# uncbiag/DeepAtlas

Hardware: AMD Instinct MI355X
Metric: training volumes/sec at 160x192x160 fp32; Dice vs CPU ref (higher is better)
Workload: dtype f32; 1 GPU; seg-only UNet_light + softmax-Dice + Adam training step, batch 2/GPU, 160x192x160 fp32 (BASELINE configs[1]); global_batch=2, n_classes=32, parallelism=dp1, matrix_precision=fp32_split, hip_graph=False, matrix_arithmetic_bits=22

## Files before the change

deepatlas_amd/csrc/conv3d_mfma.hip:

```cpp
#include "common.h"
#include "conv3d_internal.h"
#include "split_f16.h"

#include "conv3d_stage.h"
#ifndef DA_BF16_SMAP
#ifndef DA_BF16_SMAP2
#define DA_BF16_SMAP2 0
#endif
#define DA_BF16_SMAP 1
#endif
#ifndef DA_SP_LB
#define DA_SP_LB 1
#endif
#ifndef DA_RPB4
#define DA_RPB4 0
#endif
#ifndef DA_PIN
#define DA_PIN 1
#endif

namespace {


template <int CK, int NREP, bool MASKED = false, int STATS = 0, bool BF = false, bool PRO = false, bool SP = false, int S2F = 0, bool PAIR = false, bool HB = false>
__global__ void __launch_bounds__(256, 2) conv3_mfma_fwd_kernel(FwdP p) {
    static_assert(!HB || (BF && !SP), "bf16 activation storage: bf16 matrix mode only");
    static_assert(STATS != 2 || (SP && NREP == 1 && !PRO), "BatchNorm-backward sums: the split mode's one-N-tile data gradient");
    static_assert((S2F != 0) == MASKED, "the tap-masked (stride-2) variants and only they address X / dX through the space-to-depth view");
    static_assert(!PAIR || (SP && NREP == 1 && !PRO), "paired staging: split mode, one N-tile, no input prologue");
    static_assert(!SP || (BF && !MASKED && CK == 8), "split mode: dense bf16 K = 32 kernels on 8-channel chunks");
    constexpr int NP = SP ? 2 : 1;
    constexpr bool RAW = HB && BF && !SP && !PRO && !MASKED && S2F == 0;
    extern __shared__ __attribute__((aligned(16))) float lds[];
    constexpr bool K32 = BF && !MASKED;
    using AElem = std::conditional_t<BF, short, float>;
    using Frag = std::conditional_t<SP, f16x8, std::conditional_t<K32, bf16x8, std::conditional_t<BF, s16x4, f32x4>>>;
    constexpr int EB = BF ? 2 : 4;
    constexpr int TZ = 4, HZ = TZ + 2;
    constexpr int NSTEPS = K32 ? (CK == 16 ? 14 : 7) : (27 * CK + 15) / 16;
    constexpr int NIT = StageGeom<CK, HZ>::NIT;
    constexpr int PRE = MASKED ? (NREP == 1 ? NIT : 4) : ((NREP <= 2) ? NIT : (NREP == 3 ? (NIT < 4 ? NIT : 4) : 0));
    static_assert(!PRO || (PRE == NIT && !MASKED), "the prologue variant keeps the whole next tile in registers");
    const int lane = threadIdx.x & 63;
    const int wave = __builtin_amdgcn_readfirstlane((int)(threadIdx.x >> 6));
    const int i = lane & 15, g = lane >> 4;
    const int nt0 = blockIdx.y * NREP;
    const unsigned long long clk0 = __builtin_readcyclecounter(), rt0 = __builtin_amdgcn_s_memrealtime();
    const int nchunks = (p.C1 + p.C2) / CK;
    const TileWalk tw = tile_walk(p.ntiles);
    const int nitems = tw.cnt * nchunks;
    if (nitems <= 0) {
        if (STATS) for (int c = threadIdx.x; c < NREP * 16; c += 256) { const int co = blockIdx.y * NREP * 16 + c; if (co < p.Cout) { p.stats_partial[((size_t)blockIdx.x * 2) * p.Cout + co] = 0.0; p.stats_partial[((size_t)blockIdx.x * 2 + 1) * p.Cout + co] = 0.0; } }
        return;
    }
// ... 32 lines not shown
                    if constexpr (NIT > B2) { float4 tmp[NIT - B2]; stage_load_s2d<CK, HZ, B2, NIT, HB>(tmp, p.in1, p.s2in, cbase, n, z0, y0, x0, p.D, p.H, p.W); stage_write<CK, HZ, B2, NIT, BF, SP>(lds, tmp); }
                }
            } else {
            { float4 tmp[B1 - PRE]; stage_load<CK, HZ, PRE, B1, HB, RAW>(tmp, src, Cs, choff, n, z0, y0, x0, p.D, p.H, p.W); stage_write<CK, HZ, PRE, B1, BF, SP, 0, RAW>(lds, tmp); }
            if constexpr (B2 > B1) { float4 tmp[B2 - B1]; stage_load<CK, HZ, B1, B2, HB, RAW>(tmp, src, Cs, choff, n, z0, y0, x0, p.D, p.H, p.W); stage_write<CK, HZ, B1, B2, BF, SP, 0, RAW>(lds, tmp); }
            if constexpr (NIT > B2) { float4 tmp[NIT - B2]; stage_load<CK, HZ, B2, NIT, HB, RAW>(tmp, src, Cs, choff, n, z0, y0, x0, p.D, p.H, p.W); stage_write<CK, HZ, B2, NIT, BF, SP, 0, RAW>(lds, tmp); }
            }
        }
    };

    f32x4 acc[TY][NREP];
#pragma unroll
    for (int r = 0; r < TY; ++r)
#pragma unroll
        for (int nn = 0; nn < NREP; ++nn) acc[r][nn] = (f32x4){0.f, 0.f, 0.f, 0.f};

    float st1[STATS ? NREP : 1][4], st2[STATS ? NREP : 1][4];
#pragma unroll
    for (int nn = 0; nn < (STATS ? NREP : 1); ++nn)
#pragma unroll
        for (int j = 0; j < 4; ++j) { st1[nn][j] = 0.f; st2[nn][j] = 0.f; }
    double dsum1 = 0.0, dsum2 = 0.0;
    double* sred = reinterpret_cast<double*>(reinterpret_cast<char*>(lds) + (size_t)StageGeom<CK, HZ>::TOTAL * 4 * EB * NP);
    int tiles_done = 0;
    auto stats_flush = [&]() {
        if constexpr (STATS) {
#pragma unroll
            for (int nn = 0; nn < NREP; ++nn)
#pragma unroll
                for (int j = 0; j < 4; ++j) {
                    double a = (double)st1[nn][j], b = (double)st2[nn][j];
                    a += __shfl_xor(a, 1); b += __shfl_xor(b, 1);
                    a += __shfl_xor(a, 2); b += __shfl_xor(b, 2);
                    a += __shfl_xor(a, 4); b += __shfl_xor(b, 4);
                    a += __shfl_xor(a, 8); b += __shfl_xor(b, 8);
                    if ((lane & 15) == 0) {
                        const int c = nn * 16 + 4 * (lane >> 4) + j;
                        sred[(wave * 2 + 0) * (NREP * 16) + c] = a;
                        sred[(wave * 2 + 1) * (NREP * 16) + c] = b;
                    }
                    st1[nn][j] = 0.f; st2[nn][j] = 0.f;
                }
            __syncthreads();
            if ((int)threadIdx.x < NREP * 16) {
                const int c = threadIdx.x;
#pragma unroll
                for (int w = 0; w < 4; ++w) { dsum1 += sred[(w * 2 + 0) * (NREP * 16) + c]; dsum2 += sred[(w * 2 + 1) * (NREP * 16) + c]; }
            }
            __syncthreads();
        }
    };
    float4 pre[PRE > 0 ? PRE : 1];
    float4 pre2[PAIR ? PRE : 1];
    unsigned vm = 0;
    float4 psc = make_float4(1.f, 1.f, 1.f, 1.f), psf = make_float4(0.f, 0.f, 0.f, 0.f); float pslope = -1.f;
    auto load_pro = [&](int item) {
        if constexpr (PRO) {
            int n, z0, y0, x0, ch;
            item_coords(item, n, z0, y0, x0, ch);
            const int cbase = ch * CK;
            const bool first = cbase < p.C1;
            const int cofs = (first ? cbase : cbase - p.C1) + ((int)threadIdx.x % StageGeom<CK, HZ>::Q) * 4;
            psc = *reinterpret_cast<const float4*>((first ? p.ps1 : p.ps2) + cofs);
            psf = *reinterpret_cast<const float4*>((first ? p.pt1 : p.pt2) + cofs);
            pslope = first ? p.pslope1 : p.pslope2;
// ... 76 lines not shown
        else if constexpr (BF) return __builtin_amdgcn_mfma_f32_16x16x16bf16_1k(b, a, c, 0, 0, 0);
        else return c;
    };
    constexpr int LB = SP ? (NREP == 1 ? DA_SP_LB : 1) : (NREP == 1) ? 4 : ((NREP == 2 && !STATS) ? 2 : 1);
    constexpr int RB = LB + 1;
    constexpr int TAIL = SP ? 2 : 5;
    constexpr int PRO_DELAY = SP ? 1 : 3;
    constexpr bool PRO_IN = PRO && NREP == 1;
    static_assert(!PRO || NSTEPS - TAIL + PRO_DELAY <= NSTEPS, "prologue arithmetic must fall inside the K loop");
    Frag bq[RB][NREP][NP], nb[LB][NREP][NP];
    if constexpr (!MASKED) {
#pragma unroll
        for (int t = 0; t < LB; ++t)
#pragma unroll
            for (int nn = 0; nn < NREP; ++nn)
#pragma unroll
                for (int pl = 0; pl < NP; ++pl) nb[t][nn][pl] = wb(0, t, nn, pl);
    }
    const int a4 = g;
    float bvv[NREP][4];
#pragma unroll
    for (int nn = 0; nn < NREP; ++nn)
#pragma unroll
        for (int j = 0; j < 4; ++j) { const int co = (nt0 + nn) * 16 + 4 * a4 + j; bvv[nn][j] = (p.bias && co < p.Cout) ? p.bias[co] : 0.f; }

    auto item_body = [&](int item, auto PHC) {
        constexpr int PH = decltype(PHC)::value;
        int n, z0, y0, x0, ch;
        item_coords(0, n, z0, y0, x0, ch);
        const bool has_next = PH == 1 ? true : (item + 1 < nitems);
        const bool last = (ch == nchunks - 1);
        if constexpr (SP) {
            if (Ecur != Eacc) {
                if (ch != 0) {
                    const float f = da_acc_factor(Ecur - Eacc);
#pragma unroll
                    for (int r = 0; r < TY; ++r)
#pragma unroll
                        for (int nn = 0; nn < NREP; ++nn) acc[r][nn] = acc[r][nn] * f;
                }
                Eacc = Ecur;
            }
        }

        if constexpr (MASKED) {
            const Frag* wch = reinterpret_cast<const Frag*>(p.wp) + ((size_t)ch * NSTEPS * p.NT + nt0) * 64 + lane;
            if (has_next && !(p.ablate & 1)) issue_stage(1, pre);
// ... 160 lines not shown
#pragma unroll
                for (int nn = 0; nn < NREP; ++nn)
#pragma unroll
                    for (int r = 0; r < HALF; ++r) acc[HALF + r][nn] = mma_bf(acc[HALF + r][nn], A1[r], bq[s % RB][nn][0]);
            } else {
#pragma unroll
            for (int m = 0; m < 4; ++m) {
#pragma unroll
                for (int nn = 0; nn < NREP; ++nn)
#pragma unroll
                    for (int r = 0; r < HALF; ++r)
                        acc[HALF + r][nn] = __builtin_amdgcn_mfma_f32_16x16x4f32(bq[s % RB][nn][0][m], A1[r][m], acc[HALF + r][nn], 0, 0, 0);
                if (DA_PIN) __builtin_amdgcn_sched_barrier(0);
            }
            }
        }
        }

        {
            const int z = z0 + wave;
            const int x = x0 + i;
            const bool do_ep = last && !(p.ablate & 2);
            const float inv1 = SP ? da_pow2(-(Ecur / 2)) : 1.f, inv2 = SP ? da_pow2(-(Ecur - Ecur / 2)) : 1.f;
            float4 yq[STATS == 2 ? TY : 1], bsc = make_float4(0.f, 0.f, 0.f, 0.f), bsf = bsc, bmu = bsc;
            if constexpr (STATS == 2) {
                const int cq = nt0 * 16 + 4 * a4;
                const bool cokq = do_ep && (cq + 3 < p.Cout) && z < p.D && x < p.W;
                const __amdgpu_buffer_rsrc_t ry = da_rsrc_n<false>(p.bst_y, n, (long long)p.D * p.H * p.W * p.Cs1);
#pragma unroll
                for (int r = 0; r < TY; ++r) {
                    const unsigned off = ((unsigned)((z * p.H + (y0 + r)) * p.W + x) * (unsigned)p.Cs1 + (unsigned)cq) * 4u;
                    yq[r] = da_buf_load4(ry, (cokq && y0 + r < p.H) ? off : 0xFFFFFFFFu);
                }
                const __amdgpu_buffer_rsrc_t rp = da_rsrc(p.bst_par, (unsigned)(4 * p.Cs1 * 4));
                const unsigned po = (do_ep && cq + 3 < p.Cout) ? (unsigned)(cq * 4) : 0xFFFFFFFFu;
                bmu = da_buf_load4(rp, po);
                bsc = da_buf_load4(rp, po == 0xFFFFFFFFu ? po : po + (unsigned)(2 * p.Cs1 * 4));
                bsf = da_buf_load4(rp, po == 0xFFFFFFFFu ? po : po + (unsigned)(3 * p.Cs1 * 4));
            }
            if (do_ep) {
#pragma unroll
                for (int nn = 0; nn < NREP; ++nn) {
#pragma unroll
                    for (int r = 0; r < TY; ++r) {
                        float t0 = acc[r][nn][0], t1 = acc[r][nn][1], t2 = acc[r][nn][2], t3 = acc[r][nn][3];
                        if constexpr (SP) { t0 = t0 * inv1 * inv2; t1 = t1 * inv1 * inv2; t2 = t2 * inv1 * inv2; t3 = t3 * inv1 * inv2; }
                        const float v0 = t0 + bvv[nn][0], v1 = t1 + bvv[nn][1], v2 = t2 + bvv[nn][2], v3 = t3 + bvv[nn][3];
                        if constexpr (STATS == 2) {
                            const float m = (z < p.D && y0 + r < p.H && x < p.W) ? 1.f : 0.f;
                            const float4 yv = yq[r];
                            const float d0 = m * v0 * da_act_grad(yv.x * bsc.x + bsf.x, p.bst_slope), d1 = m * v1 * da_act_grad(yv.y * bsc.y + bsf.y, p.bst_slope);
                            const float d2 = m * v2 * da_act_grad(yv.z * bsc.z + bsf.z, p.bst_slope), d3 = m * v3 * da_act_grad(yv.w * bsc.w + bsf.w, p.bst_slope);
                            st1[nn][0] += d0; st1[nn][1] += d1; st1[nn][2] += d2; st1[nn][3] += d3;
                            st2[nn][0] += d0 * (yv.x - bmu.x); st2[nn][1] += d1 * (yv.y - bmu.y); st2[nn][2] += d2 * (yv.z - bmu.z); st2[nn][3] += d3 * (yv.w - bmu.w);
                        } else if (STATS) {
                            const float m = (z < p.D && y0 + r < p.H && x < p.W) ? 1.f : 0.f;
                            st1[nn][0] += m * v0; st1[nn][1] += m * v1; st1[nn][2] += m * v2; st1[nn][3] += m * v3;
                            st2[nn][0] += m * v0 * v0; st2[nn][1] += m * v1 * v1; st2[nn][2] += m * v2 * v2; st2[nn][3] += m * v3 * v3;
                        }
                        acc[r][nn] = (f32x4){da_act(v0, p.slope), da_act(v1, p.slope), da_act(v2, p.slope), da_act(v3, p.slope)};
                        if constexpr (STATS) __builtin_amdgcn_sched_barrier(0);
                    }
                }
            }
#pragma unroll
            for (int nn = 0; nn < NREP; ++nn) {
                const int cb = (nt0 + nn) * 16;
                const bool first = cb < p.Cs1;
                float* dbase = first ? p.out1 : p.out2;
                const int Cd = first ? p.Cs1 : p.Cs2;
                const int cd = cb - (first ? 0 : p.Cs1) + 4 * a4;
                const bool cok = do_ep && (cb + 4 * a4 + 3 < p.Cout) && z < p.D && x < p.W;
                constexpr bool scattered = (S2F == 2);
                if constexpr (S2F == 2) {
                    {
                        const int rr = cb / p.s2out.cin, c0 = cb - rr * p.s2out.cin + 4 * a4;
                        const int zs = 2 * z + ((rr >> 2) & 1), xs = 2 * x + (rr & 1), ry = (rr >> 1) & 1;
                        const long long sample0 = (long long)p.s2out.D0 * p.s2out.H0 * p.s2out.W0 * p.s2out.cin;
                        const __amdgpu_buffer_rsrc_t r0 = da_rsrc_n<HB>(p.out1, n, sample0);
                        const bool ok0 = cok && zs < p.s2out.D0 && xs < p.s2out.W0;
#pragma unroll
                        for (int r = 0; r < TY; ++r) {
                            const int ys = 2 * (y0 + r) + ry;
                            const unsigned off = ((unsigned)((zs * p.s2out.H0 + ys) * p.s2out.W0 + xs) * (unsigned)(p.s2out.cin) + (unsigned)(c0)) * (unsigned)(HbEl<HB>::ES);
// ... 1368 lines not shown
    size_t pk = 0;
    if (Cin % 8 == 0) { const size_t a = packed_bytes(Cin, Cout, Cin % 16 == 0 ? 16 : 8); if (a > pk) pk = a; const size_t b = packed_bytes(Cin, Cout, 8); if (b > pk) pk = b; }
    if (Cout % 8 == 0) { const size_t a = packed_bytes(Cout, Cin, Cout % 16 == 0 ? 16 : 8); if (a > pk) pk = a; }
    size_t part = 0;
    if (Cin % 8 == 0) { part = wgrad_plan(N, D, H, W, Cin, 0, Cout).partial_bytes; const size_t pr = wgrad_plan(N, D, H, W, Cin, 0, Cout, true, true, true).partial_bytes; if (pr > part) part = pr; }
    if (Cin <= 4 && Cout <= 32) part = da_align((size_t)kScBlocksFwd * 27 * Cin * Cout * sizeof(float));
    if (Cout <= 4 && Cin <= 32) { const size_t sw = da_align((size_t)(kScBlocksFwd + 1) * 27 * Cin * Cout * sizeof(float)); if (sw > part) part = sw; }
    return pk + tile_table_bytes(N, D, H, W) + part + wg_tile_table_bytes(N, D, H, W);
}

bool da_conv3_mfma_fwd_supported(int C1, int C2, int Cout, int stride, int Cs1, int Cs2) {
    if (stride != 1) return false;
    if (pick_ck(C1, C2) == 0) return false;
    if (Cout < 8) return false;
    if (Cout % 4 != 0) return false;
    if (Cs1 < 0) { Cs1 = Cout; Cs2 = 0; }
    if (Cs2 > 0 && (Cs1 % 16 != 0 || Cs2 % 4 != 0)) return false;
    if ((unsigned long long)Cs1 % 4 != 0) return false;
    return true;
}

template <int CK, int NREP, bool MASKED = false, int STATS = 0, bool BF = false, bool PRO = false, bool SP = false, int S2F = 0, bool PAIR = false, bool HB = false>
static int launch_fwd_mfma(const FwdP& p, int gy, hipStream_t st) {
    const size_t shm = (size_t)6 * HY * HX * CK * (BF ? 2 : 4) * (SP ? 2 : 1) + (STATS ? (size_t)4 * 2 * NREP * 16 * sizeof(double) : 0) + (SP ? 16 : 0);
    auto kern = conv3_mfma_fwd_kernel<CK, NREP, MASKED, STATS, BF, PRO, SP, S2F, PAIR, HB>;
    static bool attr_set = false;
    if (!attr_set) {
        hipError_t e = hipFuncSetAttribute(reinterpret_cast<const void*>(kern), hipFuncAttributeMaxDynamicSharedMemorySize, (int)shm);
        if (e != hipSuccess) return (int)e;
        attr_set = true;
    }
    { static int occ = -1; if (occ < 0) { occ = getenv("DA_OCC") ? 1 : 0; if (occ) { int nb = 0; (void)hipOccupancyMaxActiveBlocksPerMultiprocessor(&nb, kern, 256, shm); fprintf(stderr, "[occ] <%d,%d,M%d,S%d,BF%d,PRO%d,SP%d> lds %zu B -> %d workgroups per CU\n", CK, NREP, (int)MASKED, (int)STATS, (int)BF, (int)PRO, (int)SP, shm, nb); } } }
    static unsigned long long* dclk = nullptr; static int want = -1;
    if (want < 0) { want = getenv("DA_CLK") ? 1 : 0; if (want) (void)hipMalloc(&dclk, 64 + 1024 * 16); }
    FwdP q = p; q.clk = want ? dclk : nullptr;
    if (want) { const unsigned long long init[6] = {0, 0, ~0ull, 0, ~0ull, 0}; (void)hipMemcpyAsync(dclk, init, 48, hipMemcpyHostToDevice, st); (void)hipStreamSynchronize(st); }
    hipLaunchKernelGGL(kern, dim3(p.nblocks, gy), dim3(256), shm, st, q);
    if (want) {
        unsigned long long h[6]; (void)hipStreamSynchronize(st); (void)hipMemcpy(h, dclk, 48, hipMemcpyDeviceToHost);
        fprintf(stderr, "[clk] cycles %llu realtime %llu -> %.0f MHz; grid %d x %d: starts span %.1f us, ends span %.1f us, first start -> last end %.1f us\n", h[0], h[1],
                (double)h[0] / (double)h[1] * 100.0, p.nblocks, gy, (h[3] - h[2]) * 0.01, (h[5] - h[4]) * 0.01, (h[5] - h[2]) * 0.01);
        if (getenv("DA_CLK_DUMP")) {
            static unsigned long long rec[2048];
            const int nb = p.nblocks < 1024 ? p.nblocks : 1024;
            (void)hipMemcpy(rec, dclk + 8, (size_t)nb * 16, hipMemcpyDeviceToHost);
            for (int b = 0; b < nb; ++b) fprintf(stderr, "[blk] %d xcc %llu hwid %08llx life_us %.1f\n", b, (rec[2 * b] >> 32) & 15, rec[2 * b] & 0xffffffffull, rec[2 * b + 1] * 0.01);
        }
// ... 11 lines not shown
        float* h = (float*)malloc(2 * kProMaxC * sizeof(float));
        for (int i = 0; i < kProMaxC; ++i) { h[i] = 1.f; h[kProMaxC + i] = 0.f; }
        e = hipMemcpy(buf, h, 2 * kProMaxC * sizeof(float), hipMemcpyHostToDevice);
        free(h);
        if (e != hipSuccess) return (int)e;
    }
    *ones = buf; *zeros = buf + kProMaxC;
    return 0;
}

static int pro_slopes(const DaPro* pro, int C2, float* s1, float* s2) {
    const float a = pro->s1 ? pro->slope1 : -1.f, b = (C2 > 0 && pro->s2) ? pro->slope2 : -1.f;
    if (a >= 1.f || b >= 1.f) return 1;
    *s1 = a < 0.f ? 1.f : a; *s2 = b < 0.f ? 1.f : b;
    return 0;
}

static int conv3_mfma_fwd_impl(const float* in1, int C1, const float* in2, int C2, const float* w_tio, int w_is_flipped_tr,
                               const float* bias, float* out1, int Cs1, float* out2, int Cs2,
                               int N, int D, int H, int W, int Cout, int stride, float slope,
                               void* ws, size_t ws_bytes, hipStream_t st, int s2d_cin, double* stats_partial, int* stats_nparts, const DaPro* pro, const DaS2dFuse* s2f,
                               int cout0, int CoutW, bool hb);

struct BstState { const float* y; const float* par; float slope; };
static thread_local BstState g_bst = {nullptr, nullptr, -1.f};

struct PrepackState { int mode; const float* w; char* buf[2]; size_t bytes[2]; int next, used; };
static thread_local PrepackState g_pp = {0, nullptr, {nullptr, nullptr}, {0, 0}, 0, 0};
static thread_local PackJobs* g_pp_collect = nullptr;
static thread_local int g_pp_ncollect = 0;

int da_conv3_mfma_fwd(const float* in1, int C1, const float* in2, int C2, const float* w_tio, int w_is_flipped_tr,
                      const float* bias, float* out1, int Cs1, float* out2, int Cs2,
                      int N, int D, int H, int W, int Cout, int stride, float slope,
                      void* ws, size_t ws_bytes, hipStream_t st, int s2d_cin, double* stats_partial, int* stats_nparts, const DaPro* pro, const DaS2dFuse* s2f, int act_bf16) {
    if (act_bf16 && da_matrix_mode() != 1) return DA_ERR_UNSUPPORTED;
    struct PpReset { ~PpReset() { if (g_pp.mode == 1) g_pp.mode = 0; } } pp_reset;
    if (g_pp.mode && g_pp.w != w_tio) g_pp.mode = 0;
    if (da_matrix_mode() == 2 && w_is_flipped_tr && s2d_cin == 0 && !stats_partial && !pro && Cs2 > 0 && Cs1 == 32 && Cs2 == 16 && Cout == 48 &&
        pick_ck(C1, C2) != 0) {
        int rc = conv3_mfma_fwd_impl(in1, C1, in2, C2, w_tio, 1, bias, out1, 32, nullptr, 0, N, D, H, W, 32, stride, slope, ws, ws_bytes, st, 0, nullptr, nullptr,
                                     nullptr, nullptr, 0, Cout, false);
        if (rc) return rc;
        return conv3_mfma_fwd_impl(in1, C1, in2, C2, w_tio, 1, bias ? bias + 32 : nullptr, out2, 16, nullptr, 0, N, D, H, W, 16, stride, slope, ws, ws_bytes, st, 0,
                                   nullptr, nullptr, nullptr, nullptr, 32, Cout, false);
    }
    return conv3_mfma_fwd_impl(in1, C1, in2, C2, w_tio, w_is_flipped_tr, bias, out1, Cs1, out2, Cs2, N, D, H, W, Cout, stride, slope, ws, ws_bytes, st, s2d_cin,
                               stats_partial, stats_nparts, pro, s2f, 0, Cout, act_bf16 != 0);
// ... 2 lines not shown
static int conv3_mfma_fwd_impl(const float* in1, int C1, const float* in2, int C2, const float* w_tio, int w_is_flipped_tr,
                               const float* bias, float* out1, int Cs1, float* out2, int Cs2,
                               int N, int D, int H, int W, int Cout, int stride, float slope,
                               void* ws, size_t ws_bytes, hipStream_t st, int s2d_cin, double* stats_partial, int* stats_nparts, const DaPro* pro, const DaS2dFuse* s2f,
                               int cout0, int CoutW, bool hb) {
    (void)stride;
    const int Cin = C1 + C2;
    int CK = pick_ck(C1, C2);
    if (!CK) return DA_ERR_UNSUPPORTED;
    if (pro && (s2d_cin > 0 || w_is_flipped_tr || Cin > kProMaxC)) return DA_ERR_UNSUPPORTED;
    if (s2d_cin > 0 && !s2f) return DA_ERR_UNSUPPORTED;
    const bool split = da_matrix_mode() == 2 && s2d_cin == 0;
    const bool bf = da_matrix_mode() == 1;
    if (split) CK = 8;
    {
        const unsigned long long vox4 = (unsigned long long)D * H * W * 4ull;
        const int cmax = (C1 > C2 ? C1 : C2) > (Cs1 > Cs2 ? Cs1 : Cs2) ? (C1 > C2 ? C1 : C2) : (Cs1 > Cs2 ? Cs1 : Cs2);
        if (vox4 * (unsigned long long)cmax >= 0xFFFFFFF0ull) return DA_ERR_UNSUPPORTED;
    }
    const int NT = (Cout + 15) / 16;
    int NREP = pick_nrep(NT);
    if ((bf || split || pro) && NREP > 2) NREP = 2;
    const bool want_bst = g_bst.y != nullptr && split && stats_partial != nullptr;
    if (want_bst) NREP = 1;
    {
        const long long tiles = (long long)N * ((D + 3) / 4) * ((H + TY - 1) / TY) * ((W + TX - 1) / TX);
        if (s2d_cin == 0 && NREP > 1 && !want_bst) {
            auto cost = [&](int nrep) {
                const int g = (NT + nrep - 1) / nrep;
                long long nb = 512 / g; if (nb < 1) nb = 1; if (nb > tiles) nb = tiles;
                return (double)((tiles + nb - 1) / nb) * nrep * (nrep == 1 ? 1.08 : 1.0);
            };
            if (cost(1) < cost(NREP)) NREP = 1;
        }
    }
    const int gy = (NT + NREP - 1) / NREP, NTpad = gy * NREP;
    const int pkmode = split ? 3 : bf ? (s2d_cin > 0 ? 1 : 2) : 0;
    const int NSTEPS = pkmode >= 2 ? (CK == 16 ? 14 : 7) : (27 * CK + 15) / 16;
    const size_t pk = packed_bytes(Cin, Cout, CK);
    char* opbase = reinterpret_cast<char*>(ws);
    int pp_mode = 0;
    if (g_pp.mode && split) {
        const int idx = g_pp.next++;
        if (idx < 2 && g_pp.buf[idx] && g_pp.bytes[idx] >= pk + tile_table_bytes(N, D, H, W)) { opbase = g_pp.buf[idx]; pp_mode = g_pp.mode; }
        else if (g_pp.mode == 2) return DA_ERR_WS_SMALL;
    } else if (g_pp.mode == 2) return DA_ERR_UNSUPPORTED;
    if (!pp_mode && ws_bytes < pk + tile_table_bytes(N, D, H, W)) return DA_ERR_WS_SMALL;
// ... 32 lines not shown
    }
    { static int abl = -1; if (abl < 0) { const char* e = getenv("DA_ABLATE"); abl = e ? atoi(e) : 0; } p.ablate = abl; }
    {
        int nblk = 512 / gy; if (nblk < 1) nblk = 1; if (nblk > p.ntiles) nblk = p.ntiles;
        if (nblk >= 8) nblk &= ~7;
        p.nblocks = nblk;
    }
    p.s2in = S2dSrc{0, 0, 0, 0}; p.s2out = S2dSrc{0, 0, 0, 0};
    if (s2d_cin > 0) (w_is_flipped_tr ? p.s2out : p.s2in) = S2dSrc{s2d_cin, s2f->D0, s2f->H0, s2f->W0};
    p.stats_partial = stats_partial;
    if (stats_nparts) *stats_nparts = 0;
    p.ps1 = p.pt1 = p.ps2 = p.pt2 = nullptr; p.pslope1 = p.pslope2 = -1.f;
    p.wexp = wexp;
    if (pro) {
        const float *ones, *zeros;
        if (const int rc = pro_identity(&ones, &zeros)) return rc;
        if (pro_slopes(pro, C2, &p.pslope1, &p.pslope2)) return DA_ERR_UNSUPPORTED;
        p.ps1 = pro->s1 ? pro->s1 : ones; p.pt1 = pro->s1 ? pro->t1 : zeros;
        p.ps2 = (C2 > 0 && pro->s2) ? pro->s2 : ones; p.pt2 = (C2 > 0 && pro->s2) ? pro->t2 : zeros;
    }
    if (split) {
        if (stats_partial && stats_nparts) *stats_nparts = p.nblocks;
        if (want_bst) {
            if (!(NREP == 1 && !pro && Cs2 == 0 && gy <= 2)) return DA_ERR_UNSUPPORTED;
            p.bst_y = g_bst.y; p.bst_par = g_bst.par; p.bst_slope = g_bst.slope;
            return launch_fwd_mfma<8, 1, false, 2, true, false, true>(p, gy, st);
        }
        if (NREP == 1 && !pro && C1 % 16 == 0 && C2 % 16 == 0)
            return stats_partial ? launch_fwd_mfma<8, 1, false, true, true, false, true, 0, true>(p, gy, st)
                                 : launch_fwd_mfma<8, 1, false, false, true, false, true, 0, true>(p, gy, st);
#define DA_SP_CASE(nr) if (NREP == nr) return stats_partial ? (pro ? launch_fwd_mfma<8, nr, false, true, true, true, true>(p, gy, st) : launch_fwd_mfma<8, nr, false, true, true, false, true>(p, gy, st)) \
                                                              : (pro ? launch_fwd_mfma<8, nr, false, false, true, true, true>(p, gy, st) : launch_fwd_mfma<8, nr, false, false, true, false, true>(p, gy, st))
        DA_SP_CASE(1); DA_SP_CASE(2);
#undef DA_SP_CASE
        return DA_ERR_UNSUPPORTED;
    }
    if (stats_partial && p.maskmode == 0 && (CK == 16 || CK == 8) && NREP <= 2) {
        if (stats_nparts) *stats_nparts = p.nblocks;
#define DA_ST_CASE(ck, nr) if (CK == ck && NREP == nr) return pro ? (hb ? launch_fwd_mfma<ck, nr, false, true, true, true, false, 0, false, true>(p, gy, st) : bf ? launch_fwd_mfma<ck, nr, false, true, true, true>(p, gy, st) : launch_fwd_mfma<ck, nr, false, true, false, true>(p, gy, st)) \
                                                                  : (hb ? launch_fwd_mfma<ck, nr, false, true, true, false, false, 0, false, true>(p, gy, st) : bf ? launch_fwd_mfma<ck, nr, false, true, true>(p, gy, st) : launch_fwd_mfma<ck, nr, false, true>(p, gy, st))
        DA_ST_CASE(16, 1); DA_ST_CASE(16, 2); DA_ST_CASE(8, 1); DA_ST_CASE(8, 2);
#undef DA_ST_CASE
    }
    if (pro) {
#define DA_PRO_CASE(ck, nr) if (CK == ck && NREP == nr) return hb ? launch_fwd_mfma<ck, nr, false, false, true, true, false, 0, false, true>(p, gy, st) : bf ? launch_fwd_mfma<ck, nr, false, false, true, true>(p, gy, st) : launch_fwd_mfma<ck, nr, false, false, false, true>(p, gy, st)
        DA_PRO_CASE(16, 1); DA_PRO_CASE(16, 2); DA_PRO_CASE(8, 1); DA_PRO_CASE(8, 2);
#undef DA_PRO_CASE
        return DA_ERR_UNSUPPORTED;
    }
// ... 351 lines not shown
        DA_LAUNCH_CHECK();
        return 0;
    };
    g_pp_collect = &jobs; g_pp_ncollect = 0;
    int rc = 0;
    for (int i = 0; i < n && !rc; ++i) {
        if (g_pp_ncollect + 2 > kPackJobsMax) rc = flush();
        if (!rc) rc = da_conv3d_k3_prepack(w_tio[i], C1[i], C2[i], Cout[i], dgrad[i], N[i], D[i], H[i], W[i], b0[i], n0[i], b1[i], n1[i], &used[i], stream);
    }
    if (!rc) rc = flush();
    g_pp_collect = nullptr; g_pp_ncollect = 0;
    return rc;
}

extern "C" int da_conv3d_k3_dgrad_bst(const float* dy, const float* w_tio, float* dx1, int C1, float* dx2, int C2, int N, int D, int H, int W, int Cout,
                                      const float* y, const float* stats4, float slope, double* bst, int bst_cap, int* bst_n,
                                      void* ws, size_t ws_bytes, void* stream) {
    if (bst_n) *bst_n = 0;
    if (!dy || !w_tio || !dx1 || !y || !stats4 || !bst || !bst_n || C1 <= 0 || C2 < 0 || (C2 > 0 && !dx2) || N <= 0 || Cout <= 0) return DA_ERR_BADARG;
    if (da_matrix_mode() != 2 || bst_cap < 512) return DA_ERR_UNSUPPORTED;
    if (C2 == 0) {
        if (C1 > 32 || C1 % 4 != 0 || (C1 > 16 && C1 % 16 != 0) || !da_conv3_mfma_fwd_supported(Cout, 0, C1, 1, C1, 0)) return DA_ERR_UNSUPPORTED;
        if (ws_bytes < da_conv3_mfma_ws_bytes(N, D, H, W, C1, Cout, 1)) return DA_ERR_WS_SMALL;
        g_bst = BstState{y, stats4, slope};
        const int rc = da_conv3_mfma_fwd(dy, Cout, nullptr, 0, w_tio, 1, nullptr, dx1, C1, nullptr, 0, N, D, H, W, C1, 1, -1.f, ws, ws_bytes, (hipStream_t)stream, 0, bst, bst_n);
        g_bst = BstState{nullptr, nullptr, -1.f};
        return rc;
    }
    if (C1 != 32 || C2 % 16 != 0 || C2 > 16 || !da_conv3_mfma_fwd_supported(Cout, 0, C1 + C2, 1, C1, C2) || pick_ck(Cout, 0) == 0) return DA_ERR_UNSUPPORTED;
    if (ws_bytes < da_conv3_mfma_ws_bytes(N, D, H, W, C1 + C2, Cout, 1)) return DA_ERR_WS_SMALL;
    struct PpReset { ~PpReset() { if (g_pp.mode == 1) g_pp.mode = 0; } } pp_reset;
    if (g_pp.mode && g_pp.w != w_tio) g_pp.mode = 0;
    g_bst = BstState{y, stats4, slope};
    int rc = conv3_mfma_fwd_impl(dy, Cout, nullptr, 0, w_tio, 1, nullptr, dx1, C1, nullptr, 0, N, D, H, W, C1, 1, -1.f, ws, ws_bytes, (hipStream_t)stream, 0, bst, bst_n,
                                 nullptr, nullptr, 0, C1 + C2, false);
    g_bst = BstState{nullptr, nullptr, -1.f};
    if (rc) { *bst_n = 0; return rc; }
    rc = conv3_mfma_fwd_impl(dy, Cout, nullptr, 0, w_tio, 1, nullptr, dx2, C2, nullptr, 0, N, D, H, W, C2, 1, -1.f, ws, ws_bytes, (hipStream_t)stream, 0, nullptr, nullptr,
                             nullptr, nullptr, C1, C1 + C2, false);
    if (rc) *bst_n = 0;
    return rc;
}
```

deepatlas_amd/lib/network_factory/unets.py:

```python
import torch
import torch.nn as nn

from ... import ops

from .modules import (SegBlock as convBlock, SegUpBlock as deconvBlock, HeadConv, MaxPool2, DownConv, UpsampleTrilinear2,
                      UNetEncBlock, UNetDecBlock, get_activation_function)


def init_conv_weights(m):
    classname = m.__class__.__name__
    if classname.find('Conv') != -1:
        if not m.weight is None:
            ops.init_into(m.weight, nn.init.xavier_normal_)
        if not m.bias is None:
            m.bias.data.zero_()


def UNet_generator(encoders, decoders, act='ReLU', upsample=False, maxpool=True, res=False):

    class UNetTemplate(nn.Module):
        def __init__(self, in_channel, n_classes, bias=False, BN=False):
            super(UNetTemplate, self).__init__()
            self.register_forward_hook(ops.flush_batches_tracked)
            self.in_channel = in_channel
# ... 52 lines not shown
            temp = []
            for i, enc in enumerate(self.encoders):
                y = x
                blks = list(enc)
                into_pool = (ops.LAZY_BN and self.maxpool and not self.res and i < self.levels - 1 and getattr(blks[-1], 'supports_lazy', False)
                             and getattr(blks[-1], 'batchnorm', False) and getattr(blks[-1], 'stride', 1) == 1 and isinstance(blks[-1], convBlock))
                for k, blk in enumerate(blks):
                    nxt = blks[k + 1] if k + 1 < len(blks) else None
                    y = blk(y, lazy_out=True) if (lazy_ok(blk, nxt) or (nxt is None and into_pool)) else blk(y)
                x = (y + x) if self.res else y
                if i < self.levels - 1:
                    if self.maxpool:
                        if isinstance(x, ops.LazyAct):
                            skip, x = ops.MaxPool2SkipFn.apply(x.raw, x.scale, x.shift, x.slope)
                        else:
                            skip, x = ops.MaxPool2SkipFn.apply(x)
                        temp.append(skip)
                    else:
                        temp.append(x)
                        x = self.down_samplers[i](x)
            for j, dec in enumerate(self.decoders):
                blocks = list(dec)
                up = self.up_samplers[j]
                x = up(x, lazy_out=True) if (ops.LAZY_BN_UPSAMPLER and not self.res and lazy_ok(up, blocks[0])) else up(x)
                skip = temp.pop()
                nxt = blocks[1] if len(blocks) > 1 else None
                y = blocks[0](x, skip, lazy_out=True) if lazy_ok(blocks[0], nxt) else blocks[0](x, skip)
                for k in range(1, len(blocks)):
                    nxt = blocks[k + 1] if k + 1 < len(blocks) else None
                    y = blocks[k](y, lazy_out=True) if lazy_ok(blocks[k], nxt) else blocks[k](y)
                x = (ops.materialize_logits(y) + x) if self.res else y
            return x

    return UNetTemplate


class UNet(nn.Module):

    def __init__(self, in_channel, n_classes, bias=False, BN=False):
        self.in_channel = in_channel
        self.n_classes = n_classes
        super(UNet, self).__init__()
        self.register_forward_hook(ops.flush_batches_tracked)
        self.ec0 = self.encoder(self.in_channel, 32, bias=bias, batchnorm=BN)
        self.ec1 = self.encoder(32, 64, bias=bias, batchnorm=BN)
        self.ec2 = self.encoder(64, 64, bias=bias, batchnorm=BN)
        self.ec3 = self.encoder(64, 128, bias=bias, batchnorm=BN)
# ... 56 lines not shown
```

deepatlas_amd/ops.py:

```python
import os

import torch
from torch.autograd import Function

from . import _native as nat
from ._native import call, call_supported, ptr, stream, workspace


def ndhwc(x):
    nat.require_cuda(x)
    if x.dtype != torch.float32 and x.dtype != torch.bfloat16:
        raise nat.NativeError('deepatlas_amd kernels take fp32 tensors (bf16 for the activations of the bf16 storage mode); got %s' % x.dtype)
    xp = x.permute(0, 2, 3, 4, 1)
    return xp if xp.is_contiguous() else xp.contiguous()


def ncdhw(t):
    return t.permute(0, 4, 1, 2, 3)


def _empty(shape, like, dtype=torch.float32):
    return torch.empty(shape, dtype=dtype, device=like.device)


ACT_STORAGE_MODES = ('fp32', 'bf16')
ACT_STORAGE = 'fp32'


def set_activation_storage(mode):
    global ACT_STORAGE
    if mode not in ACT_STORAGE_MODES:
        raise ValueError("activation storage must be one of %r, got %r" % (ACT_STORAGE_MODES, mode))
    prev, ACT_STORAGE = ACT_STORAGE, mode
    global LAZY_BN_UPSAMPLER
    LAZY_BN_UPSAMPLER = mode == 'bf16'
    return prev


def _act_dtype(channels=None):
    if ACT_STORAGE == 'bf16' and (channels is None or (channels >= 8 and channels % 4 == 0)):
        return torch.bfloat16
    return torch.float32


class A(object):
    __slots__ = ('t', 'out')

    def __init__(self, t, out=False):
        self.t, self.out = t, out


def O(t):
    return A(t, True)


_TWIN_PATTERN = {'da_conv1x1_fwd': (1, 0), 'da_conv1x1_fwd_pro': (1, 0), 'da_conv1x1_dgrad': (0, 1), 'da_conv1x1_wgrad': (1, 0),
                 'da_conv1x1_wgrad_pro': (1, 0)}
BF16_FORCE_BRIDGE = False
# ... 454 lines not shown
            return ent[1]
    w_tio = torch.empty((K3, Cin, Cout), dtype=torch.float32, device=weight.device)
    call(_TIO_ENTRY[kind], ptr(weight.detach().contiguous()), ptr(w_tio), a_, b_, K3, stream())
    if stamp is not None:
        try:
            weight._da_tio = (stamp, w_tio)
        except AttributeError:
            pass
    return w_tio


def grad_from_tio(dw_tio, kind, shape, acc=None):
    a_, b_ = int(shape[0]), int(shape[1])
    K3 = int(dw_tio.shape[0])
    if acc is not None:
        call(_TIO_BACK[kind] + '_acc', ptr(dw_tio), ptr(acc), a_, b_, K3, stream())
        return None
    dw = torch.empty(tuple(shape), dtype=torch.float32, device=dw_tio.device)
    call(_TIO_BACK[kind], ptr(dw_tio), ptr(dw), a_, b_, K3, stream())
    return dw


LAZY_BN = True
LAZY_BN_UPSAMPLER = False


class LazyAct(object):
    __slots__ = ('raw', 'scale', 'shift', 'slope')

    def __init__(self, raw, scale, shift, slope):
        self.raw, self.scale, self.shift, self.slope = raw, scale, shift, float(slope)

    @property
    def shape(self):
        return self.raw.shape

    def materialize(self):
        return ApplyAffineActFn.apply(self.raw, self.scale, self.shift, self.slope)


def materialize(x):
    return x.materialize() if isinstance(x, LazyAct) else x


class ApplyAffineActFn(Function):

    @staticmethod
# ... 1378 lines not shown
```

Measured before the change: 100.3 volumes/s.

## Enable lazy BN upsampler in split mode and two-N-tile fused BN-backward stats

Extends the split-mode data-gradient kernel that fuses the BatchNorm-backward sums so it also handles two output-channel tiles (NREP=2). Per-tile statistic registers are spilled to LDS and the y reads are processed in row blocks to limit register pressure. The change also turns on the lazy BN upsampler path for fp32_split when the upsampler has 32 output channels, which lets the decoder concat conv run the fused BN-backward with NREP=2. It removes a separate normalisation and statistics pass, at the cost of extra LDS traffic and more registers held in the epilogue.

After: 100.5 volumes/s (median of 6 runs). About the same (+0.2%).

```diff
diff --git a/deepatlas_amd/csrc/conv3d_mfma.hip b/deepatlas_amd/csrc/conv3d_mfma.hip
--- a/deepatlas_amd/csrc/conv3d_mfma.hip
+++ b/deepatlas_amd/csrc/conv3d_mfma.hip
@@ -15,6 +15,9 @@
 #ifndef DA_RPB4
 #define DA_RPB4 0
 #endif
+#ifndef DA_BST_YB
+#define DA_BST_YB 4
+#endif
 #ifndef DA_PIN
 #define DA_PIN 1
 #endif
@@ -25,11 +28,13 @@
 template <int CK, int NREP, bool MASKED = false, int STATS = 0, bool BF = false, bool PRO = false, bool SP = false, int S2F = 0, bool PAIR = false, bool HB = false>
 __global__ void __launch_bounds__(256, 2) conv3_mfma_fwd_kernel(FwdP p) {
     static_assert(!HB || (BF && !SP), "bf16 activation storage: bf16 matrix mode only");
-    static_assert(STATS != 2 || (SP && NREP == 1 && !PRO), "BatchNorm-backward sums: the split mode's one-N-tile data gradient");
+    static_assert(STATS != 2 || (SP && NREP <= 2 && !PRO), "BatchNorm-backward sums: the split mode's one- and two-N-tile data gradients");
     static_assert((S2F != 0) == MASKED, "the tap-masked (stride-2) variants and only they address X / dX through the space-to-depth view");
     static_assert(!PAIR || (SP && NREP == 1 && !PRO), "paired staging: split mode, one N-tile, no input prologue");
     static_assert(!SP || (BF && !MASKED && CK == 8), "split mode: dense bf16 K = 32 kernels on 8-channel chunks");
     constexpr int NP = SP ? 2 : 1;
+    constexpr bool STL = STATS == 2 && NREP == 2;
+    constexpr int YB = STL ? DA_BST_YB : TY;
     constexpr bool RAW = HB && BF && !SP && !PRO && !MASKED && S2F == 0;
     extern __shared__ __attribute__((aligned(16))) float lds[];
     constexpr bool K32 = BF && !MASKED;
@@ -108,9 +113,27 @@
         for (int j = 0; j < 4; ++j) { st1[nn][j] = 0.f; st2[nn][j] = 0.f; }
     double dsum1 = 0.0, dsum2 = 0.0;
     double* sred = reinterpret_cast<double*>(reinterpret_cast<char*>(lds) + (size_t)StageGeom<CK, HZ>::TOTAL * 4 * EB * NP);
+    float4* stl = reinterpret_cast<float4*>(reinterpret_cast<char*>(lds) + (size_t)StageGeom<CK, HZ>::TOTAL * 4 * EB * NP + (STATS ? (size_t)4 * 2 * NREP * 16 * sizeof(double) : 0) + (SP ? 16 : 0));
+    auto st_load = [&](int nn) {
+        if constexpr (STL) {
+            const float4 a = stl[nn * 256 + threadIdx.x], b = stl[(NREP + nn) * 256 + threadIdx.x];
+            st1[nn][0] = a.x; st1[nn][1] = a.y; st1[nn][2] = a.z; st1[nn][3] = a.w;
+            st2[nn][0] = b.x; st2[nn][1] = b.y; st2[nn][2] = b.z; st2[nn][3] = b.w;
+        }
+    };
+    auto st_store = [&](int nn) {
+        if constexpr (STL) {
+            stl[nn * 256 + threadIdx.x] = make_float4(st1[nn][0], st1[nn][1], st1[nn][2], st1[nn][3]);
+            stl[(NREP + nn) * 256 + threadIdx.x] = make_float4(st2[nn][0], st2[nn][1], st2[nn][2], st2[nn][3]);
+        }
+    };
+#pragma unroll
+    for (int nn = 0; nn < (STL ? NREP : 0); ++nn) st_store(nn);
     int tiles_done = 0;
     auto stats_flush = [&]() {
         if constexpr (STATS) {
+#pragma unroll
+            for (int nn = 0; nn < (STL ? NREP : 0); ++nn) st_load(nn);
 #pragma unroll
             for (int nn = 0; nn < NREP; ++nn)
 #pragma unroll
@@ -127,6 +150,8 @@
                     }
                     st1[nn][j] = 0.f; st2[nn][j] = 0.f;
                 }
+#pragma unroll
+            for (int nn = 0; nn < (STL ? NREP : 0); ++nn) st_store(nn);
             __syncthreads();
             if ((int)threadIdx.x < NREP * 16) {
                 const int c = threadIdx.x;
@@ -249,7 +274,7 @@
 #pragma unroll
     for (int nn = 0; nn < NREP; ++nn)
 #pragma unroll
-        for (int j = 0; j < 4; ++j) { const int co = (nt0 + nn) * 16 + 4 * a4 + j; bvv[nn][j] = (p.bias && co < p.Cout) ? p.bias[co] : 0.f; }
+        for (int j = 0; j < 4; ++j) { const int co = (nt0 + nn) * 16 + 4 * a4 + j; bvv[nn][j] = (STATS != 2 && p.bias && co < p.Cout) ? p.bias[co] : 0.f; }
 
     auto item_body = [&](int item, auto PHC) {
         constexpr int PH = decltype(PHC)::value;
@@ -456,44 +481,49 @@
             const int x = x0 + i;
             const bool do_ep = last && !(p.ablate & 2);
             const float inv1 = SP ? da_pow2(-(Ecur / 2)) : 1.f, inv2 = SP ? da_pow2(-(Ecur - Ecur / 2)) : 1.f;
-            float4 yq[STATS == 2 ? TY : 1], bsc = make_float4(0.f, 0.f, 0.f, 0.f), bsf = bsc, bmu = bsc;
-            if constexpr (STATS == 2) {
-                const int cq = nt0 * 16 + 4 * a4;
-                const bool cokq = do_ep && (cq + 3 < p.Cout) && z < p.D && x < p.W;
-                const __amdgpu_buffer_rsrc_t ry = da_rsrc_n<false>(p.bst_y, n, (long long)p.D * p.H * p.W * p.Cs1);
-#pragma unroll
-                for (int r = 0; r < TY; ++r) {
-                    const unsigned off = ((unsigned)((z * p.H + (y0 + r)) * p.W + x) * (unsigned)p.Cs1 + (unsigned)cq) * 4u;
-                    yq[r] = da_buf_load4(ry, (cokq && y0 + r < p.H) ? off : 0xFFFFFFFFu);
-                }
-                const __amdgpu_buffer_rsrc_t rp = da_rsrc(p.bst_par, (unsigned)(4 * p.Cs1 * 4));
-                const unsigned po = (do_ep && cq + 3 < p.Cout) ? (unsigned)(cq * 4) : 0xFFFFFFFFu;
-                bmu = da_buf_load4(rp, po);
-                bsc = da_buf_load4(rp, po == 0xFFFFFFFFu ? po : po + (unsigned)(2 * p.Cs1 * 4));
-                bsf = da_buf_load4(rp, po == 0xFFFFFFFFu ? po : po + (unsigned)(3 * p.Cs1 * 4));
-            }
-            if (do_ep) {
-#pragma unroll
-                for (int nn = 0; nn < NREP; ++nn) {
-#pragma unroll
-                    for (int r = 0; r < TY; ++r) {
-                        float t0 = acc[r][nn][0], t1 = acc[r][nn][1], t2 = acc[r][nn][2], t3 = acc[r][nn][3];
-                        if constexpr (SP) { t0 = t0 * inv1 * inv2; t1 = t1 * inv1 * inv2; t2 = t2 * inv1 * inv2; t3 = t3 * inv1 * inv2; }
-                        const float v0 = t0 + bvv[nn][0], v1 = t1 + bvv[nn][1], v2 = t2 + bvv[nn][2], v3 = t3 + bvv[nn][3];
-                        if constexpr (STATS == 2) {
-                            const float m = (z < p.D && y0 + r < p.H && x < p.W) ? 1.f : 0.f;
-                            const float4 yv = yq[r];
-                            const float d0 = m * v0 * da_act_grad(yv.x * bsc.x + bsf.x, p.bst_slope), d1 = m * v1 * da_act_grad(yv.y * bsc.y + bsf.y, p.bst_slope);
-                            const float d2 = m * v2 * da_act_grad(yv.z * bsc.z + bsf.z, p.bst_slope), d3 = m * v3 * da_act_grad(yv.w * bsc.w + bsf.w, p.bst_slope);
-                            st1[nn][0] += d0; st1[nn][1] += d1; st1[nn][2] += d2; st1[nn][3] += d3;
-                            st2[nn][0] += d0 * (yv.x - bmu.x); st2[nn][1] += d1 * (yv.y - bmu.y); st2[nn][2] += d2 * (yv.z - bmu.z); st2[nn][3] += d3 * (yv.w - bmu.w);
-                        } else if (STATS) {
-                            const float m = (z < p.D && y0 + r < p.H && x < p.W) ? 1.f : 0.f;
-                            st1[nn][0] += m * v0; st1[nn][1] += m * v1; st1[nn][2] += m * v2; st1[nn][3] += m * v3;
-                            st2[nn][0] += m * v0 * v0; st2[nn][1] += m * v1 * v1; st2[nn][2] += m * v2 * v2; st2[nn][3] += m * v3 * v3;
+#pragma unroll
+            for (int nn = 0; nn < NREP; ++nn) {
+#pragma unroll
+                for (int rb = 0; rb < TY; rb += YB) {
+                    float4 yq[STATS == 2 ? YB : 1], bsc = make_float4(0.f, 0.f, 0.f, 0.f), bsf = bsc, bmu = bsc;
+                    if constexpr (STATS == 2) {
+                        const int cq = (nt0 + nn) * 16 + 4 * a4;
+                        const bool cokq = do_ep && (cq + 3 < p.Cout) && z < p.D && x < p.W;
+                        const __amdgpu_buffer_rsrc_t ry = da_rsrc_n<false>(p.bst_y, n, (long long)p.D * p.H * p.W * p.Cs1);
+#pragma unroll
+                        for (int r = rb; r < rb + YB; ++r) {
+                            const unsigned off = ((unsigned)((z * p.H + (y0 + r)) * p.W + x) * (unsigned)p.Cs1 + (unsigned)cq) * 4u;
+                            yq[r - rb] = da_buf_load4(ry, (cokq && y0 + r < p.H) ? off : 0xFFFFFFFFu);
                         }
-                        acc[r][nn] = (f32x4){da_act(v0, p.slope), da_act(v1, p.slope), da_act(v2, p.slope), da_act(v3, p.slope)};
-                        if constexpr (STATS) __builtin_amdgcn_sched_barrier(0);
+                        const __amdgpu_buffer_rsrc_t rp = da_rsrc(p.bst_par, (unsigned)(4 * p.Cs1 * 4));
+                        const unsigned po = (do_ep && cq + 3 < p.Cout) ? (unsigned)(cq * 4) : 0xFFFFFFFFu;
+                        bmu = da_buf_load4(rp, po);
+                        bsc = da_buf_load4(rp, po == 0xFFFFFFFFu ? po : po + (unsigned)(2 * p.Cs1 * 4));
+                        bsf = da_buf_load4(rp, po == 0xFFFFFFFFu ? po : po + (unsigned)(3 * p.Cs1 * 4));
+                    }
+                    if (do_ep) {
+                        if constexpr (STL) if (rb == 0) st_load(nn);
+#pragma unroll
+                        for (int r = rb; r < rb + YB; ++r) {
+                            float t0 = acc[r][nn][0], t1 = acc[r][nn][1], t2 = acc[r][nn][2], t3 = acc[r][nn][3];
+                            if constexpr (SP) { t0 = t0 * inv1 * inv2; t1 = t1 * inv1 * inv2; t2 = t2 * inv1 * inv2; t3 = t3 * inv1 * inv2; }
+                            const float v0 = t0 + bvv[nn][0], v1 = t1 + bvv[nn][1], v2 = t2 + bvv[nn][2], v3 = t3 + bvv[nn][3];
+                            if constexpr (STATS == 2) {
+                                const float m = (z < p.D && y0 + r < p.H && x < p.W) ? 1.f : 0.f;
+                                const float4 yv = yq[r - rb];
+                                const float d0 = m * v0 * da_act_grad(yv.x * bsc.x + bsf.x, p.bst_slope), d1 = m * v1 * da_act_grad(yv.y * bsc.y + bsf.y, p.bst_slope);
+                                const float d2 = m * v2 * da_act_grad(yv.z * bsc.z + bsf.z, p.bst_slope), d3 = m * v3 * da_act_grad(yv.w * bsc.w + bsf.w, p.bst_slope);
+                                st1[nn][0] += d0; st1[nn][1] += d1; st1[nn][2] += d2; st1[nn][3] += d3;
+                                st2[nn][0] += d0 * (yv.x - bmu.x); st2[nn][1] += d1 * (yv.y - bmu.y); st2[nn][2] += d2 * (yv.z - bmu.z); st2[nn][3] += d3 * (yv.w - bmu.w);
+                            } else if (STATS) {
+                                const float m = (z < p.D && y0 + r < p.H && x < p.W) ? 1.f : 0.f;
+                                st1[nn][0] += m * v0; st1[nn][1] += m * v1; st1[nn][2] += m * v2; st1[nn][3] += m * v3;
+                                st2[nn][0] += m * v0 * v0; st2[nn][1] += m * v1 * v1; st2[nn][2] += m * v2 * v2; st2[nn][3] += m * v3 * v3;
+                            }
+                            acc[r][nn] = (f32x4){da_act(v0, p.slope), da_act(v1, p.slope), da_act(v2, p.slope), da_act(v3, p.slope)};
+                            if constexpr (STATS) __builtin_amdgcn_sched_barrier(0);
+                        }
+                        if constexpr (STL) if (rb + YB == TY) st_store(nn);
                     }
                 }
             }
@@ -1908,7 +1938,8 @@
 
 template <int CK, int NREP, bool MASKED = false, int STATS = 0, bool BF = false, bool PRO = false, bool SP = false, int S2F = 0, bool PAIR = false, bool HB = false>
 static int launch_fwd_mfma(const FwdP& p, int gy, hipStream_t st) {
-    const size_t shm = (size_t)6 * HY * HX * CK * (BF ? 2 : 4) * (SP ? 2 : 1) + (STATS ? (size_t)4 * 2 * NREP * 16 * sizeof(double) : 0) + (SP ? 16 : 0);
+    const size_t shm = (size_t)6 * HY * HX * CK * (BF ? 2 : 4) * (SP ? 2 : 1) + (STATS ? (size_t)4 * 2 * NREP * 16 * sizeof(double) : 0) + (SP ? 16 : 0)
+                     + (STATS == 2 && NREP == 2 ? (size_t)2 * NREP * 256 * 16 : 0);
     auto kern = conv3_mfma_fwd_kernel<CK, NREP, MASKED, STATS, BF, PRO, SP, S2F, PAIR, HB>;
     static bool attr_set = false;
     if (!attr_set) {
@@ -1966,8 +1997,8 @@
                                void* ws, size_t ws_bytes, hipStream_t st, int s2d_cin, double* stats_partial, int* stats_nparts, const DaPro* pro, const DaS2dFuse* s2f,
                                int cout0, int CoutW, bool hb);
 
-struct BstState { const float* y; const float* par; float slope; };
-static thread_local BstState g_bst = {nullptr, nullptr, -1.f};
+struct BstState { const float* y; const float* par; float slope; int nrep; };
+static thread_local BstState g_bst = {nullptr, nullptr, -1.f, 1};
 
 struct PrepackState { int mode; const float* w; char* buf[2]; size_t bytes[2]; int next, used; };
 static thread_local PrepackState g_pp = {0, nullptr, {nullptr, nullptr}, {0, 0}, 0, 0};
@@ -2016,7 +2047,7 @@
     int NREP = pick_nrep(NT);
     if ((bf || split || pro) && NREP > 2) NREP = 2;
     const bool want_bst = g_bst.y != nullptr && split && stats_partial != nullptr;
-    if (want_bst) NREP = 1;
+    if (want_bst) NREP = g_bst.nrep;
     {
         const long long tiles = (long long)N * ((D + 3) / 4) * ((H + TY - 1) / TY) * ((W + TX - 1) / TX);
         if (s2d_cin == 0 && NREP > 1 && !want_bst) {
@@ -2095,9 +2126,10 @@
     if (split) {
         if (stats_partial && stats_nparts) *stats_nparts = p.nblocks;
         if (want_bst) {
-            if (!(NREP == 1 && !pro && Cs2 == 0 && gy <= 2)) return DA_ERR_UNSUPPORTED;
+            if (!((NREP == 1 || NREP == 2) && !pro && Cs2 == 0 && gy * NREP <= 2)) return DA_ERR_UNSUPPORTED;
             p.bst_y = g_bst.y; p.bst_par = g_bst.par; p.bst_slope = g_bst.slope;
-            return launch_fwd_mfma<8, 1, false, 2, true, false, true>(p, gy, st);
+            return NREP == 2 ? launch_fwd_mfma<8, 2, false, 2, true, false, true>(p, gy, st)
+                             : launch_fwd_mfma<8, 1, false, 2, true, false, true>(p, gy, st);
         }
         if (NREP == 1 && !pro && C1 % 16 == 0 && C2 % 16 == 0)
             return stats_partial ? launch_fwd_mfma<8, 1, false, true, true, false, true, 0, true>(p, gy, st)
@@ -2495,19 +2527,19 @@
     if (C2 == 0) {
         if (C1 > 32 || C1 % 4 != 0 || (C1 > 16 && C1 % 16 != 0) || !da_conv3_mfma_fwd_supported(Cout, 0, C1, 1, C1, 0)) return DA_ERR_UNSUPPORTED;
         if (ws_bytes < da_conv3_mfma_ws_bytes(N, D, H, W, C1, Cout, 1)) return DA_ERR_WS_SMALL;
-        g_bst = BstState{y, stats4, slope};
+        g_bst = BstState{y, stats4, slope, 1};
         const int rc = da_conv3_mfma_fwd(dy, Cout, nullptr, 0, w_tio, 1, nullptr, dx1, C1, nullptr, 0, N, D, H, W, C1, 1, -1.f, ws, ws_bytes, (hipStream_t)stream, 0, bst, bst_n);
-        g_bst = BstState{nullptr, nullptr, -1.f};
+        g_bst = BstState{nullptr, nullptr, -1.f, 1};
         return rc;
     }
     if (C1 != 32 || C2 % 16 != 0 || C2 > 16 || !da_conv3_mfma_fwd_supported(Cout, 0, C1 + C2, 1, C1, C2) || pick_ck(Cout, 0) == 0) return DA_ERR_UNSUPPORTED;
     if (ws_bytes < da_conv3_mfma_ws_bytes(N, D, H, W, C1 + C2, Cout, 1)) return DA_ERR_WS_SMALL;
     struct PpReset { ~PpReset() { if (g_pp.mode == 1) g_pp.mode = 0; } } pp_reset;
     if (g_pp.mode && g_pp.w != w_tio) g_pp.mode = 0;
-    g_bst = BstState{y, stats4, slope};
+    g_bst = BstState{y, stats4, slope, 2};
     int rc = conv3_mfma_fwd_impl(dy, Cout, nullptr, 0, w_tio, 1, nullptr, dx1, C1, nullptr, 0, N, D, H, W, C1, 1, -1.f, ws, ws_bytes, (hipStream_t)stream, 0, bst, bst_n,
                                  nullptr, nullptr, 0, C1 + C2, false);
-    g_bst = BstState{nullptr, nullptr, -1.f};
+    g_bst = BstState{nullptr, nullptr, -1.f, 1};
     if (rc) { *bst_n = 0; return rc; }
     rc = conv3_mfma_fwd_impl(dy, Cout, nullptr, 0, w_tio, 1, nullptr, dx2, C2, nullptr, 0, N, D, H, W, C2, 1, -1.f, ws, ws_bytes, (hipStream_t)stream, 0, nullptr, nullptr,
                              nullptr, nullptr, C1, C1 + C2, false);
diff --git a/deepatlas_amd/lib/network_factory/unets.py b/deepatlas_amd/lib/network_factory/unets.py
--- a/deepatlas_amd/lib/network_factory/unets.py
+++ b/deepatlas_amd/lib/network_factory/unets.py
@@ -98,7 +98,7 @@
             for j, dec in enumerate(self.decoders):
                 blocks = list(dec)
                 up = self.up_samplers[j]
-                x = up(x, lazy_out=True) if (ops.LAZY_BN_UPSAMPLER and not self.res and lazy_ok(up, blocks[0])) else up(x)
+                x = up(x, lazy_out=True) if (ops.lazy_bn_upsampler(getattr(getattr(up, 'deconv', None), 'out_channels', None)) and not self.res and lazy_ok(up, blocks[0])) else up(x)
                 skip = temp.pop()
                 nxt = blocks[1] if len(blocks) > 1 else None
                 y = blocks[0](x, skip, lazy_out=True) if lazy_ok(blocks[0], nxt) else blocks[0](x, skip)
diff --git a/deepatlas_amd/ops.py b/deepatlas_amd/ops.py
--- a/deepatlas_amd/ops.py
+++ b/deepatlas_amd/ops.py
@@ -32,8 +32,6 @@
     if mode not in ACT_STORAGE_MODES:
         raise ValueError("activation storage must be one of %r, got %r" % (ACT_STORAGE_MODES, mode))
     prev, ACT_STORAGE = ACT_STORAGE, mode
-    global LAZY_BN_UPSAMPLER
-    LAZY_BN_UPSAMPLER = mode == 'bf16'
     return prev
 
 
@@ -534,7 +532,13 @@
 
 
 LAZY_BN = True
-LAZY_BN_UPSAMPLER = False
+LAZY_BN_UPSAMPLER = None
+
+
+def lazy_bn_upsampler(channels=None):
+    if LAZY_BN_UPSAMPLER is not None:
+        return bool(LAZY_BN_UPSAMPLER)
+    return ACT_STORAGE == 'bf16' or (_matrix_mode == 'fp32_split' and channels == 32)
 
 
 class LazyAct(object):
```
